# ZhengyiLuo/PULSE

Hardware: AMD Instinct MI355X
Metric: env-steps/sec through PPO update (higher is better)
Workload: dtype f32; 1 GPU; cfg2: 4096 SMPL-humanoid envs/GPU x horizon 32, imitation obs/reward/reset + PPO (actor+critic MLP [1024, 512], minibatch 16384 x 6 mini-epochs); num_envs_per_gpu=4096, horizon=32, global_batch=131072, parallelism=dp1, reference_motion=HBM-resident motion library (1024 clips), queried every step

## Files before the change

pulse_amd/csrc/build.py:

```python
import argparse
import os
import subprocess
from concurrent.futures import ThreadPoolExecutor

HERE = os.path.dirname(os.path.abspath(__file__))
ROOT = os.path.dirname(os.path.dirname(HERE))
INCLUDE = os.path.join(ROOT, "include")
LIB = os.path.join(HERE, "libpulse_hip.so")
ARCH = "gfx950"

NO_CONTRACT = ["-ffp-contract=off"]
NO_PACKED_F32 = ["-fno-slp-vectorize", "-fno-vectorize"]
LLVM_BIN = "/opt/rocm/lib/llvm/bin"
SOURCES = [
    ("capi.cpp", []),
    ("rot_ops.hip", NO_CONTRACT),
    ("env_step.hip", NO_CONTRACT),
    ("amp_obs.hip", NO_CONTRACT),
    ("task_step.hip", NO_CONTRACT),
    ("traj_step.hip", NO_CONTRACT),
    ("motion_state.hip", NO_CONTRACT),
    ("motion_build.hip", NO_CONTRACT),
    ("eval_metrics.hip", NO_CONTRACT),
    ("rollout_ops.hip", NO_CONTRACT),
    ("gae.hip", NO_CONTRACT),
    ("gemm_f32.hip", ["-mllvm", "-amdgpu-mfma-vgpr-form"]),
    ("gemm_x3.hip", ["-mllvm", "-amdgpu-mfma-vgpr-form"]),
    ("gemm_api.hip", ["-mllvm", "-amdgpu-mfma-vgpr-form"]),
    ("gemm_x3p.hip", ["-mllvm", "-amdgpu-mfma-vgpr-form"]),
    ("gemm_b16.hip", ["-mllvm", "-amdgpu-mfma-vgpr-form"]),
    ("gemm_x3p_api.hip", ["-mllvm", "-amdgpu-mfma-vgpr-form"]),
    ("gemm_x3w.hip", ["-mllvm", "-pragma-unroll-threshold=4000000", "-Wno-unused-const-variable"]),
    ("gemm_x3s.hip", ["-mllvm", "-amdgpu-mfma-vgpr-form"]),
    ("learner_ops.hip", NO_CONTRACT),
    ("b16_ops.hip", NO_CONTRACT),
    ("vae_head.hip", NO_CONTRACT),
    ("mcp.hip", NO_CONTRACT),
]


def hipcc():
    for cand in (os.environ.get("HIPCC"), "/opt/rocm/bin/hipcc", "hipcc"):
        if cand and (os.path.isabs(cand) and os.path.exists(cand) or not os.path.isabs(cand)):
            return cand
    raise RuntimeError("hipcc not found")


HOST_ONLY_OBJECTS = ("capi.o",)


def llvm_bin():
    cc = hipcc()
    cands = []
    if os.path.isabs(cc):
        cands.append(os.path.join(os.path.dirname(os.path.dirname(os.path.realpath(cc))), "lib", "llvm", "bin"))
    cands.append(LLVM_BIN)
    for c in cands:
        if os.path.exists(os.path.join(c, "llvm-objdump")):
            return c
    raise RuntimeError("llvm-objdump / llvm-objcopy / clang-offload-bundler not found next to hipcc: the device-ISA audit cannot run")


def packed_f32_instructions(obj, host_only=False):
    import re
    import tempfile
    with tempfile.TemporaryDirectory() as tmp:
        fat, co = os.path.join(tmp, "fat"), os.path.join(tmp, "co")
        llvm = llvm_bin()
        r = subprocess.run([f"{llvm}/llvm-objcopy", "--dump-section", f".hip_fatbin={fat}", obj], capture_output=True, text=True)
        if r.returncode != 0 or not os.path.exists(fat) or os.path.getsize(fat) == 0:
            if host_only:
                return []
            raise RuntimeError(f"{obj}: no .hip_fatbin section could be extracted ({r.stderr.strip() or 'empty section'}); cannot audit its device ISA")
        subprocess.run([f"{llvm}/clang-offload-bundler", "--unbundle", "--type=o", f"--targets=hipv4-amdgcn-amd-amdhsa--{ARCH}",
                        f"--input={fat}", f"--output={co}"], check=True, capture_output=True)
        if not os.path.exists(co) or os.path.getsize(co) == 0:
            raise RuntimeError(f"{obj}: the offload bundle holds no {ARCH} code object; cannot audit its device ISA")
        dis = subprocess.run([f"{llvm}/llvm-objdump", "-d", co], check=True, capture_output=True, text=True).stdout
    return re.findall(r"\bv_pk_(?:mul|add|fma)_f32\b[^\n]*", dis)


def _newer(a, b):
    return (not os.path.exists(b)) or os.path.getmtime(a) > os.path.getmtime(b)


def build(force=False, verbose=False):
    cc = hipcc()
    headers = [os.path.join(HERE, f) for f in os.listdir(HERE) if f.endswith(".h")]
    headers.append(os.path.join(INCLUDE, "pulse_hip.h"))
    headers.append(os.path.abspath(__file__))
    common = ["-x", "hip", f"--offload-arch={ARCH}", "-O3", "-std=c++17", "-fPIC", "-Wall",
              "-Wno-unused-function", f"-I{INCLUDE}", f"-I{HERE}"] + NO_PACKED_F32
    jobs = []
    objs = []
    for src, extra in SOURCES:
        s = os.path.join(HERE, src)
        if not os.path.exists(s):
            continue
        o = os.path.join(HERE, os.path.splitext(src)[0] + ".o")
        objs.append(o)
        if force or _newer(s, o) or any(_newer(h, o) for h in headers):
            jobs.append((src, [cc] + common + extra + ["-c", s, "-o", o]))

    def run(job):
        name, cmd = job
        if verbose:
            print(" ".join(cmd), flush=True)
        r = subprocess.run(cmd, stdout=subprocess.PIPE, stderr=subprocess.STDOUT, text=True)
        return name, r.returncode, r.stdout

    with ThreadPoolExecutor(max_workers=max(1, min(len(jobs), os.cpu_count() or 1))) as ex:
        for name, rc, out in ex.map(run, jobs):
            if out.strip() and (verbose or rc != 0):
                print(f"--- {name} ---\n{out}", flush=True)
            if rc != 0:
                raise RuntimeError(f"hipcc failed on {name}")
    for o in objs:
        bad = packed_f32_instructions(o, host_only=os.path.basename(o) in HOST_ONLY_OBJECTS)
        if bad:
            raise RuntimeError(f"{os.path.basename(o)}: {len(bad)} packed-fp32 VALU instructions in the device code (e.g. {bad[0].strip()}); "
                               "they are unsafe beside MFMA waves on gfx950 (see the note at the top of build.py)")
    if jobs or force or not os.path.exists(LIB) or any(_newer(o, LIB) for o in objs):
        cmd = [cc, "-shared", "-fPIC", f"--offload-arch={ARCH}", "-o", LIB] + objs
        if verbose:
            print(" ".join(cmd), flush=True)
        r = subprocess.run(cmd, stdout=subprocess.PIPE, stderr=subprocess.STDOUT, text=True)
        if r.returncode != 0:
            print(r.stdout)
            raise RuntimeError("link failed")
    return LIB


if __name__ == "__main__":
    ap = argparse.ArgumentParser()
    ap.add_argument("--force", action="store_true")
    ap.add_argument("--verbose", action="store_true")
    a = ap.parse_args()
    print(build(a.force, a.verbose))
```

pulse_amd/csrc/gemm_api.hip:

```cpp
#include <cstdlib>
#include "common.h"
#include "gemm_shared.h"

namespace pulse {

__global__ void __launch_bounds__(256) reduce_slabs_kernel(const float* __restrict__ slabs, int nslab, long long slab_stride,
                                                          long long count, float* __restrict__ out, float scale) {
    for (long long i = ((long long)blockIdx.x * blockDim.x + threadIdx.x) * 4; i < count; i += (long long)gridDim.x * blockDim.x * 4) {
        if (i + 3 < count) {
            float4 s = *reinterpret_cast<const float4*>(slabs + i);
            float4 s1 = make_float4(0.f, 0.f, 0.f, 0.f), s2 = s1, s3 = s1;
            int k = 1;
            for (; k + 15 < nslab; k += 16) {
                float4 v[16];
#pragma unroll
                for (int u = 0; u < 16; ++u) v[u] = *reinterpret_cast<const float4*>(slabs + (k + u) * slab_stride + i);
#pragma unroll
                for (int u = 0; u < 16; u += 4) {
                    s.x += v[u].x; s.y += v[u].y; s.z += v[u].z; s.w += v[u].w;
                    s1.x += v[u + 1].x; s1.y += v[u + 1].y; s1.z += v[u + 1].z; s1.w += v[u + 1].w;
                    s2.x += v[u + 2].x; s2.y += v[u + 2].y; s2.z += v[u + 2].z; s2.w += v[u + 2].w;
                    s3.x += v[u + 3].x; s3.y += v[u + 3].y; s3.z += v[u + 3].z; s3.w += v[u + 3].w;
                }
            }
            for (; k + 3 < nslab; k += 4) {
                const float4 v0 = *reinterpret_cast<const float4*>(slabs + k * slab_stride + i);
                const float4 v1 = *reinterpret_cast<const float4*>(slabs + (k + 1) * slab_stride + i);
                const float4 v2 = *reinterpret_cast<const float4*>(slabs + (k + 2) * slab_stride + i);
                const float4 v3 = *reinterpret_cast<const float4*>(slabs + (k + 3) * slab_stride + i);
                s.x += v0.x; s.y += v0.y; s.z += v0.z; s.w += v0.w;
                s1.x += v1.x; s1.y += v1.y; s1.z += v1.z; s1.w += v1.w;
                s2.x += v2.x; s2.y += v2.y; s2.z += v2.z; s2.w += v2.w;
                s3.x += v3.x; s3.y += v3.y; s3.z += v3.z; s3.w += v3.w;
            }
            const int rem = nslab - k;
            if (rem == 3) {
                const float4 t0 = *reinterpret_cast<const float4*>(slabs + k * slab_stride + i);
                const float4 t1 = *reinterpret_cast<const float4*>(slabs + (k + 1) * slab_stride + i);
                const float4 t2 = *reinterpret_cast<const float4*>(slabs + (k + 2) * slab_stride + i);
                s.x += t0.x; s.y += t0.y; s.z += t0.z; s.w += t0.w;
                s.x += t1.x; s.y += t1.y; s.z += t1.z; s.w += t1.w;
                s.x += t2.x; s.y += t2.y; s.z += t2.z; s.w += t2.w;
            } else if (rem == 2) {
                const float4 t0 = *reinterpret_cast<const float4*>(slabs + k * slab_stride + i);
                const float4 t1 = *reinterpret_cast<const float4*>(slabs + (k + 1) * slab_stride + i);
                s.x += t0.x; s.y += t0.y; s.z += t0.z; s.w += t0.w;
                s.x += t1.x; s.y += t1.y; s.z += t1.z; s.w += t1.w;
            } else if (rem == 1) {
                const float4 t0 = *reinterpret_cast<const float4*>(slabs + k * slab_stride + i);
                s.x += t0.x; s.y += t0.y; s.z += t0.z; s.w += t0.w;
            }
            s.x = (s.x + s1.x) + (s2.x + s3.x); s.y = (s.y + s1.y) + (s2.y + s3.y); s.z = (s.z + s1.z) + (s2.z + s3.z); s.w = (s.w + s1.w) + (s2.w + s3.w);
            s.x *= scale; s.y *= scale; s.z *= scale; s.w *= scale;
            *reinterpret_cast<float4*>(out + i) = s;
        } else {
            for (long long e = i; e < count; ++e) {
                float s = slabs[e];
                for (int k = 1; k < nslab; ++k) s += slabs[k * slab_stride + e];
                out[e] = s * scale;
            }
        }
    }
}

__global__ void __launch_bounds__(256) colsum_partial_kernel(const float* __restrict__ X, int M, int N, int ld, int rows_per_chunk,
                                                            float* __restrict__ partial, long long ldp) {
    __shared__ float4 red[4][64];
    const int cg = threadIdx.x & 63, rl = threadIdx.x >> 6;
    const int c = blockIdx.x * 256 + cg * 4;
    const int r0 = blockIdx.y * rows_per_chunk;
    const int r1 = min(M, r0 + rows_per_chunk);
    float4 s0 = make_float4(0.f, 0.f, 0.f, 0.f), s1 = s0, s2 = s0, s3 = s0;
    if (c < N) {
        const float* p = X + c;
        int r = r0 + rl;
        for (; r + 12 < r1; r += 16) {
            const float4 a = *reinterpret_cast<const float4*>(p + (long long)r * ld);
            const float4 b = *reinterpret_cast<const float4*>(p + (long long)(r + 4) * ld);
            const float4 cc = *reinterpret_cast<const float4*>(p + (long long)(r + 8) * ld);
            const float4 d = *reinterpret_cast<const float4*>(p + (long long)(r + 12) * ld);
            s0.x += a.x; s0.y += a.y; s0.z += a.z; s0.w += a.w;
            s1.x += b.x; s1.y += b.y; s1.z += b.z; s1.w += b.w;
            s2.x += cc.x; s2.y += cc.y; s2.z += cc.z; s2.w += cc.w;
            s3.x += d.x; s3.y += d.y; s3.z += d.z; s3.w += d.w;
        }
        for (; r < r1; r += 4) {
            const float4 a = *reinterpret_cast<const float4*>(p + (long long)r * ld);
            s0.x += a.x; s0.y += a.y; s0.z += a.z; s0.w += a.w;
        }
    }
    s0.x += s1.x + s2.x + s3.x; s0.y += s1.y + s2.y + s3.y; s0.z += s1.z + s2.z + s3.z; s0.w += s1.w + s2.w + s3.w;
    red[rl][cg] = s0;
    __syncthreads();
    if (rl == 0 && c < N) {
        const float4 a = red[0][cg], b = red[1][cg], cc = red[2][cg], d = red[3][cg];
        float* o = partial + (long long)blockIdx.y * ldp + c;
        o[0] = a.x + b.x + cc.x + d.x;
        if (c + 1 < N) o[1] = a.y + b.y + cc.y + d.y;
        if (c + 2 < N) o[2] = a.z + b.z + cc.z + d.z;
        if (c + 3 < N) o[3] = a.w + b.w + cc.w + d.w;
    }
}

}

using namespace pulse;

namespace {
thread_local long long* g_dbg = nullptr;
thread_local int g_last_tile = 0;
thread_local int g_opt[16] = {0, 0, 0, 0, 0, 0, 0, 0, 0, 0, 0, 0, 0, 0, 0, 0};
}

namespace pulse { int gemm_option(int key) { return key >= 0 && key < 16 ? g_opt[key] : 0; } long long* gemm_debug_buffer() { return g_dbg; } }

namespace {
constexpr int WIDE_TILE = 256;
bool skinny_env_off() { static const bool off = [] { const char* e = getenv("PULSE_X3_SKINNY"); return e && e[0] == '0'; }(); return off; }
bool g_skinny_unavailable = false;
bool g_wide_unavailable = false;
int x3_mode() {
    static const int env = [] { const char* e = getenv("PULSE_X3_WIDE"); return e ? atoi(e) : -1; }();
    int mode = g_opt[4];
    if (mode == 0 && env >= 0) mode = env == 0 ? 1 : env == 1 ? 0 : env;
    return g_wide_unavailable ? 1 : mode;
}
bool x3_wide_tile(const GemmArgs& g, int lda, int ldb, bool akc, bool bkc) {
    const int mode = x3_mode();
    if (mode == 1 || g.M <= 128 || g.N <= 128) return false;
    if ((long long)lda * (akc ? 257 : g.kchunk + 1) >= (1LL << 28) || (long long)ldb * (bkc ? 257 : g.kchunk + 1) >= (1LL << 28) ||
        (long long)g.ldc * 257 >= (1LL << 28) || (long long)g.ldaux * 257 >= (1LL << 28))
        return false;
    if (mode == 2) return true;
    const long long z = (long long)g.batch * g.splitk;
    const long long nt = (long long)((g.M + 127) / 128) * ((g.N + 127) / 128) * z;
    const long long wt = (long long)((g.M + 255) / 256) * ((g.N + 255) / 256) * z;
    const long long rem = nt % 512;
    const double cost_narrow = 2.0 * (double)(nt / 512) + (rem == 0 ? 0.0 : rem <= 256 ? 1.5 : 2.0);
    const double kk = (double)g.kchunk < (double)g.K ? (double)g.kchunk : (double)g.K;
    const double fw = g.epi == 2 ? 45.0 : (g.epi == 0 && g.act >= 2) ? 30.0 : 8.0;
    const double wide_round = 2.0 * (0.1526 * kk + fw) / (0.0924 * kk + 5.0);
    const double cost_wide = wide_round * (double)((wt + 255) / 256);
    return cost_wide < cost_narrow;
}
}

extern "C" {

int pulse_sizeof_gemm_desc(void) { return (int)sizeof(pulse_gemm_desc); }

int pulse_gemm_set_debug_buffer(long long* device_buffer) { g_dbg = device_buffer; return PULSE_OK; }

int pulse_gemm_last_tile(void) { return g_last_tile; }
int pulse_gemm_x3_mode(void) { return x3_mode(); }

int pulse_gemm_set_option(int key, int value) {
    PULSE_REQUIRE(key >= 0 && key < 16, "pulse_gemm_set_option: bad key");
    g_opt[key] = value;
    return PULSE_OK;
}

int pulse_gemm_f32(const pulse_gemm_desc* d, pulse_stream_t s) {
    PULSE_REQUIRE(d != nullptr, "pulse_gemm_f32: null descriptor");
    PULSE_REQUIRE(d->M >= 0 && d->N >= 0 && d->K >= 0, "pulse_gemm_f32: negative size");
    if (d->M == 0 || d->N == 0 || d->batch == 0) return PULSE_OK;
    PULSE_REQUIRE(d->A && d->B && d->C, "pulse_gemm_f32: null operand");
    PULSE_REQUIRE(d->batch >= 1 && d->split_k >= 1, "pulse_gemm_f32: batch / split_k must be >= 1");
    PULSE_REQUIRE((d->lda % 4) == 0 && (d->ldb % 4) == 0, "pulse_gemm_f32: lda / ldb must be multiples of 4 floats");
    PULSE_REQUIRE((reinterpret_cast<uintptr_t>(d->A) & 15) == 0 && (reinterpret_cast<uintptr_t>(d->B) & 15) == 0,
                  "pulse_gemm_f32: A / B must be 16-byte aligned");
    PULSE_REQUIRE((d->stride_a % 4) == 0 && (d->stride_b % 4) == 0, "pulse_gemm_f32: batch strides must be multiples of 4 floats");
    const bool akc = d->a_layout == PULSE_GEMM_RED_CONTIG, bkc = d->b_layout == PULSE_GEMM_RED_CONTIG;
    PULSE_REQUIRE(!(!akc && bkc), "pulse_gemm_f32: layout combination (A out-contiguous, B reduction-contiguous) unsupported");
    const int k4 = (d->K + 3) & ~3;
    PULSE_REQUIRE(akc ? d->lda >= k4 : d->lda >= ((d->M + 3) & ~3), "pulse_gemm_f32: lda too small");
    PULSE_REQUIRE(bkc ? d->ldb >= k4 : d->ldb >= ((d->N + 3) & ~3), "pulse_gemm_f32: ldb too small");
    PULSE_REQUIRE(d->ldc >= d->N, "pulse_gemm_f32: ldc too small");
    PULSE_REQUIRE(d->epilogue >= 0 && d->epilogue <= 3 && d->activation >= 0 && d->activation <= 3, "pulse_gemm_f32: bad epilogue / activation");
    PULSE_REQUIRE(d->activation != PULSE_ACT_SILU_D || (d->C2 != nullptr && d->ldc2 >= d->N), "pulse_gemm_f32: ACT_SILU_D stores the derivative in C2");
    PULSE_REQUIRE(d->epilogue == 0 || d->activation == 0, "pulse_gemm_f32: a gradient epilogue takes no activation");
    PULSE_REQUIRE(d->epilogue == 0 || d->aux != nullptr || (d->epilogue == PULSE_EPI_RELU_GRAD && d->relu_mask != nullptr),
                  "pulse_gemm_f32: gradient epilogue needs aux (or, for relu-grad, relu_mask)");
    const bool mask_on = d->relu_mask != nullptr && ((d->epilogue == PULSE_EPI_RELU_GRAD && d->aux == nullptr) ||
                                                     (d->epilogue == PULSE_EPI_BIAS_ACT && d->activation == PULSE_ACT_RELU));
    PULSE_REQUIRE(!mask_on || (d->ld_mask >= (d->N + 3) / 4 && d->split_k == 1), "pulse_gemm_f32: relu_mask needs ld_mask >= roundup4(N) / 4 and no split-K");
    PULSE_REQUIRE(d->rowsum == nullptr || (!akc && !bkc), "pulse_gemm_f32: rowsum needs the (OUT, OUT) layouts (dW pass)");
    PULSE_REQUIRE(d->split_k == 1 || (d->epilogue == 0 && d->activation == 0 && d->bias == nullptr),
                  "pulse_gemm_f32: split-K slabs carry no epilogue");

    GemmArgs g;
    g.A = d->A; g.B = d->B; g.C = d->C; g.C2 = d->C2; g.bias = d->bias; g.aux = d->aux;
    g.M = d->M; g.N = d->N; g.K = d->K;
    g.lda = d->lda; g.ldb = d->ldb; g.ldc = d->ldc; g.ldc2 = d->ldc2; g.ldaux = d->ldaux;
    g.sA = d->stride_a; g.sB = d->stride_b; g.sC = d->stride_c; g.sC2 = d->stride_c2; g.sBias = d->stride_bias; g.sAux = d->stride_aux;
    g.batch = d->batch; g.splitk = d->split_k;
    const int bk = d->compute_type == PULSE_GEMM_COMPUTE_BF16 ? BK16 : d->compute_type == PULSE_GEMM_COMPUTE_F32X3 ? XK : BK;
    int kchunk = (d->K + d->split_k - 1) / d->split_k;
    kchunk = ((kchunk + bk - 1) / bk) * bk;
    g.kchunk = kchunk > 0 ? kchunk : bk;
    g.sSplit = d->split_stride;
    g.act = d->activation; g.epi = d->epilogue;
    g.rowsum = d->rowsum; g.sRowsum = d->stride_rowsum;
    g.mask = mask_on ? d->relu_mask : nullptr; g.ldmask = d->ld_mask; g.sMask = d->stride_mask;
    g.tiles_m = (d->M + BM - 1) / BM; g.tiles_n = (d->N + BN - 1) / BN;
    const bool half_tile = d->compute_type == PULSE_GEMM_COMPUTE_F32X3 && d->M >= 256 && g.tiles_n == 1 &&
                           (long long)g.tiles_m * d->batch * d->split_k < 384 && g_opt[2] == 0;
    if (half_tile) g.tiles_m = (d->M + 63) / 64;
    g.dbg = g_dbg;
    PULSE_REQUIRE(d->compute_type == PULSE_GEMM_COMPUTE_F32 || d->compute_type == PULSE_GEMM_COMPUTE_BF16 ||
                  d->compute_type == PULSE_GEMM_COMPUTE_F32X3, "pulse_gemm_f32: bad compute_type");
    const bool bf = d->compute_type == PULSE_GEMM_COMPUTE_BF16, x3 = d->compute_type == PULSE_GEMM_COMPUTE_F32X3;
    g.round_bf16 = bf && d->round_output_bf16 ? 1 : 0;
    PULSE_REQUIRE((long long)d->lda * (akc ? 129 : g.kchunk + 1) < (1LL << 28) && (long long)d->ldb * (bkc ? 129 : g.kchunk + 1) < (1LL << 28) &&
                  (long long)d->ldc * 129 < (1LL << 28) && (long long)d->ldaux * 129 < (1LL << 28),
                  "pulse_gemm_f32: pitch too large for 32-bit tile-relative offsets");
    auto al16 = [](const void* p, long long ld, long long st) { return (reinterpret_cast<uintptr_t>(p) & 15) == 0 && (ld % 4) == 0 && (st % 4) == 0; };
    g.vec_epi = al16(d->C, d->ldc, d->stride_c) && (d->split_stride % 4) == 0 && (!d->aux || al16(d->aux, d->ldaux, d->stride_aux)) &&
                (!d->C2 || al16(d->C2, d->ldc2, d->stride_c2)) && (!d->bias || al16(d->bias, 4, d->stride_bias));
    PULSE_REQUIRE(!mask_on || g.vec_epi, "pulse_gemm_f32: relu_mask needs 16-byte aligned C / pitches (a lane owns four columns of a mask word)");
    g_last_tile = half_tile ? 64 : 128;
    if (x3 && akc && d->N <= 96 && d->epilogue == PULSE_EPI_BIAS_ACT && d->activation <= PULSE_ACT_RELU && d->C2 == nullptr && d->split_k == 1 &&
        d->rowsum == nullptr && !mask_on && g_dbg == nullptr && g_opt[6] == 0 && !g_skinny_unavailable && !skinny_env_off() &&
        (long long)((d->M + 127) / 128) * d->batch >= 192 && (long long)((d->M + 127) / 128) * d->batch <= 256 && (long long)d->lda * 129 < (1LL << 28) &&
        (bkc ? (long long)d->ldb * 97 : (long long)d->ldb * (d->K + 1)) < (1LL << 28)) {
        const int rc = launch_gemm_x3s(g, bkc, as_stream(s));
        if (rc != kWideTileUnavailable) { g_last_tile = 96; return rc; }
        g_skinny_unavailable = true;
    }
    if (x3 && !half_tile && x3_wide_tile(g, d->lda, d->ldb, akc, bkc)) {
        const int ntail = d->N % WIDE_TILE;
        if (ntail > 0 && ntail <= 64 && d->N > WIDE_TILE && d->split_k == 1 && d->rowsum == nullptr && g_opt[5] == 0) {
            const long long tm = (d->M + WIDE_TILE - 1) / WIDE_TILE, z = d->batch;
            const long long r_all = (tm * ((d->N + WIDE_TILE - 1) / WIDE_TILE) * z + 255) / 256, r_main = (tm * (d->N / WIDE_TILE) * z + 255) / 256;
            if (r_main < r_all) {
                const int n0 = d->N - ntail;
                pulse_gemm_desc m = *d, t = *d;
                m.N = n0;
                t.N = ntail;
                t.B = bkc ? d->B + (long long)n0 * d->ldb : d->B + n0;
                t.C = d->C + n0;
                if (d->C2) t.C2 = d->C2 + n0;
                if (d->bias) t.bias = d->bias + n0;
                if (d->aux) t.aux = d->aux + n0;
                if (d->relu_mask) t.relu_mask = d->relu_mask + n0 / 4;
                const int rc_main = pulse_gemm_f32(&m, s);
                if (rc_main != PULSE_OK) return rc_main;
                const int rc_tail = pulse_gemm_f32(&t, s);
                g_last_tile = 256;
                return rc_tail;
            }
        }
        const int rc = launch_gemm_x3w(g, akc, bkc, as_stream(s));
        if (rc != kWideTileUnavailable) { g_last_tile = 256; return rc; }
        g_wide_unavailable = true;
    }
    const size_t extra_lds = (size_t)g_opt[1];
    if (x3) return launch_gemm_x3(g, akc, bkc, half_tile, extra_lds, as_stream(s));
    if (bf) return launch_gemm_bf16c(g, akc, bkc, extra_lds, as_stream(s));
    return launch_gemm_mfma32(g, akc, bkc, extra_lds, as_stream(s));
}

int pulse_reduce_slabs(const float* slabs, int32_t num_slabs, int64_t slab_stride, int64_t count, float* out, float scale,
                       pulse_stream_t s) {
    PULSE_REQUIRE(num_slabs >= 1 && count >= 0, "pulse_reduce_slabs: bad sizes");
    if (count == 0) return PULSE_OK;
    PULSE_REQUIRE(slabs && out, "pulse_reduce_slabs: null pointer");
    PULSE_REQUIRE((slab_stride % 4) == 0 && (reinterpret_cast<uintptr_t>(slabs) & 15) == 0 && (reinterpret_cast<uintptr_t>(out) & 15) == 0,
                  "pulse_reduce_slabs: 16-byte alignment required");
    long long blocks = (count / 4 + 255) / 256;
    if (blocks > 2048) blocks = 2048;
    if (blocks < 1) blocks = 1;
    hipLaunchKernelGGL(reduce_slabs_kernel, dim3((unsigned)blocks), dim3(256), 0, as_stream(s), slabs, num_slabs, slab_stride, count, out, scale);
    return check_launch("pulse_reduce_slabs");
}

int pulse_colsum_partial(const float* x, int32_t m, int32_t n, int32_t ld, int32_t num_chunks, float* partial, int64_t ld_partial,
                         pulse_stream_t s) {
    PULSE_REQUIRE(m >= 0 && n >= 0 && num_chunks >= 1, "pulse_colsum_partial: bad sizes");
    if (n == 0) return PULSE_OK;
    PULSE_REQUIRE(x && partial && ld >= ((n + 3) & ~3) && ld_partial >= n, "pulse_colsum_partial: bad pointers / pitches (ld must cover roundup4(n))");
    PULSE_REQUIRE((ld % 4) == 0 && (reinterpret_cast<uintptr_t>(x) & 15) == 0, "pulse_colsum_partial: x rows must be 16-byte aligned");
    const int rows = (m + num_chunks - 1) / num_chunks;
    hipLaunchKernelGGL(colsum_partial_kernel, dim3((unsigned)((n + 255) / 256), (unsigned)num_chunks), dim3(256), 0, as_stream(s), x, m, n, ld,
                       rows > 0 ? rows : 1, partial, (long long)ld_partial);
    return check_launch("pulse_colsum_partial");
}
}
```

pulse_amd/csrc/gemm_shared.h:

```cpp
#pragma once
#include "common.h"

namespace pulse {

typedef float f32x16 __attribute__((ext_vector_type(16)));
typedef float f32x4 __attribute__((ext_vector_type(4)));
typedef unsigned int u32x4 __attribute__((ext_vector_type(4)));

constexpr unsigned RSRC_FLAGS = 0x00020000u;

struct GemmArgs {
    const float* A; const float* B; float* C; float* C2; const float* bias; const float* aux;
    int M, N, K;
    int lda, ldb, ldc, ldc2, ldaux;
    long long sA, sB, sC, sC2, sBias, sAux;
    int batch, splitk, kchunk;
    long long sSplit;
    int act;
    int epi;
    int tiles_m, tiles_n;
    int vec_epi;
    float* rowsum; long long sRowsum;
    long long* dbg;
    int round_bf16;
    unsigned* mask; int ldmask; long long sMask;
};

__device__ __forceinline__ long long mask_word(int r, int cg, int ldmask) { return (long long)((r >> 6) * 8 + (r & 7)) * ldmask + cg; }

constexpr int BM = 128, BN = 128;
constexpr int BK = 32, BK16 = 64, XK = 16;
constexpr int CP = BN;

constexpr int kWideTileUnavailable = -1000;

__device__ __forceinline__ int slot_of(int out) { return out ^ ((out >> 3) & 7); }

__device__ __forceinline__ f32x4 buf_load(__amdgpu_buffer_rsrc_t r, int voff, int soff) {
    return __builtin_bit_cast(f32x4, __builtin_amdgcn_raw_buffer_load_b128(r, voff, soff, 0));
}
__device__ __forceinline__ void buf_store(f32x4 v, __amdgpu_buffer_rsrc_t r, int voff, int soff) {
    __builtin_amdgcn_raw_buffer_store_b128(__builtin_bit_cast(u32x4, v), r, voff, soff, 0);
}
__device__ __forceinline__ f32x4 lds_read(int byte_addr) {
    extern __shared__ __attribute__((aligned(16))) char smem_c[];
    return *reinterpret_cast<const f32x4*>(smem_c + byte_addr);
}
__device__ __forceinline__ void lds_write(int byte_addr, f32x4 v) {
    extern __shared__ __attribute__((aligned(16))) char smem_c[];
    *reinterpret_cast<f32x4*>(smem_c + byte_addr) = v;
}

typedef __bf16 bf16x2 __attribute__((ext_vector_type(2)));
typedef __bf16 bf16x8 __attribute__((ext_vector_type(8)));
typedef float f32x2 __attribute__((ext_vector_type(2)));

__device__ __forceinline__ unsigned fbits(float v) { return __builtin_bit_cast(unsigned, v); }
__device__ __forceinline__ float bitsf(unsigned v) { return __builtin_bit_cast(float, v); }
__device__ __forceinline__ unsigned pack_rn(float lo_elem, float hi_elem) {
    return __builtin_bit_cast(unsigned, __builtin_convertvector((f32x2){lo_elem, hi_elem}, bf16x2));
}

__device__ __forceinline__ float silu(float z) { return z / (1.f + __expf(-z)); }
__device__ __forceinline__ float silu_deriv(float z) {
    const float sg = 1.f / (1.f + __expf(-z));
    return sg * (1.f + z * (1.f - sg));
}
__device__ __forceinline__ float rbf(float v) { return (float)(__bf16)v; }

inline int lds_launch_status(hipError_t e, const char* what) {
    if (e != hipSuccess) return fail(PULSE_ERR_LAUNCH, "%s: LDS attribute: %s", what, hipGetErrorString(e));
    return check_launch(what);
}

int launch_gemm_mfma32(const GemmArgs& g, bool akc, bool bkc, size_t extra_lds, hipStream_t stream);
int launch_gemm_bf16c(const GemmArgs& g, bool akc, bool bkc, size_t extra_lds, hipStream_t stream);
int launch_gemm_x3(const GemmArgs& g, bool akc, bool bkc, bool half_tile, size_t extra_lds, hipStream_t stream);
int launch_gemm_x3w(const GemmArgs& g, bool akc, bool bkc, hipStream_t stream);
int launch_gemm_x3s(const GemmArgs& g, bool bkc, hipStream_t stream);

}
```

Baseline: 1.931 million env-steps/s.

## Add skinny-M split-bf16x3 MFMA kernel for small-M head weight gradients

Adds a dedicated GEMM kernel for products with M<=96 and N a multiple of 32. It targets the backward weight gradients of the small output heads. Three waves split A into three bf16 parts and stage them in double-buffered LDS, while all waves stream B through registers and issue 32x32x16 bf16 MFMAs for a six-term split product that keeps fp32-like accuracy. The dispatcher routes qualifying launches with 192-256 workgroups to this kernel and falls back if the launch fails. This replaces a generic tiled kernel that wastes most of a 128-row tile on small M, at the cost of extra code paths and a fragile dispatch condition.

```diff
diff --git a/pulse_amd/csrc/build.py b/pulse_amd/csrc/build.py
--- a/pulse_amd/csrc/build.py
+++ b/pulse_amd/csrc/build.py
@@ -32,6 +32,7 @@
     ("gemm_x3p_api.hip", ["-mllvm", "-amdgpu-mfma-vgpr-form"]),
     ("gemm_x3w.hip", ["-mllvm", "-pragma-unroll-threshold=4000000", "-Wno-unused-const-variable"]),
     ("gemm_x3s.hip", ["-mllvm", "-amdgpu-mfma-vgpr-form"]),
+    ("gemm_x3sm.hip", []),
     ("learner_ops.hip", NO_CONTRACT),
     ("b16_ops.hip", NO_CONTRACT),
     ("vae_head.hip", NO_CONTRACT),
diff --git a/pulse_amd/csrc/gemm_api.hip b/pulse_amd/csrc/gemm_api.hip
--- a/pulse_amd/csrc/gemm_api.hip
+++ b/pulse_amd/csrc/gemm_api.hip
@@ -118,6 +118,8 @@
 constexpr int WIDE_TILE = 256;
 bool skinny_env_off() { static const bool off = [] { const char* e = getenv("PULSE_X3_SKINNY"); return e && e[0] == '0'; }(); return off; }
 bool g_skinny_unavailable = false;
+bool heads_bwd_env_off() { static const bool off = [] { const char* e = getenv("PULSE_X3_HEADS_BWD"); return e && e[0] == '0'; }(); return off; }
+bool g_skinny_m_unavailable = false;
 bool g_wide_unavailable = false;
 int x3_mode() {
     static const int env = [] { const char* e = getenv("PULSE_X3_WIDE"); return e ? atoi(e) : -1; }();
@@ -227,6 +229,15 @@
         if (rc != kWideTileUnavailable) { g_last_tile = 96; return rc; }
         g_skinny_unavailable = true;
     }
+    if (x3 && !akc && !bkc && d->M <= 96 && (d->N % 32) == 0 && d->epilogue == PULSE_EPI_BIAS_ACT && d->activation == PULSE_ACT_NONE &&
+        d->bias == nullptr && d->C2 == nullptr && !mask_on && g_dbg == nullptr && g_opt[10] != 1 && !heads_bwd_env_off() && !g_skinny_m_unavailable) {
+        const long long nwg = (long long)((d->N + 127) / 128) * d->batch * d->split_k;
+        if (g_opt[10] == 2 ? nwg < (1LL << 31) : (nwg >= 192 && nwg <= 256)) {
+            const int rc = launch_gemm_x3sm(g, as_stream(s));
+            if (rc != kWideTileUnavailable) { g_last_tile = 97; return rc; }
+            g_skinny_m_unavailable = true;
+        }
+    }
     if (x3 && !half_tile && x3_wide_tile(g, d->lda, d->ldb, akc, bkc)) {
         const int ntail = d->N % WIDE_TILE;
         if (ntail > 0 && ntail <= 64 && d->N > WIDE_TILE && d->split_k == 1 && d->rowsum == nullptr && g_opt[5] == 0) {
diff --git a/pulse_amd/csrc/gemm_shared.h b/pulse_amd/csrc/gemm_shared.h
--- a/pulse_amd/csrc/gemm_shared.h
+++ b/pulse_amd/csrc/gemm_shared.h
@@ -78,5 +78,6 @@
 int launch_gemm_x3(const GemmArgs& g, bool akc, bool bkc, bool half_tile, size_t extra_lds, hipStream_t stream);
 int launch_gemm_x3w(const GemmArgs& g, bool akc, bool bkc, hipStream_t stream);
 int launch_gemm_x3s(const GemmArgs& g, bool bkc, hipStream_t stream);
+int launch_gemm_x3sm(const GemmArgs& g, hipStream_t stream);
 
 }
diff --git a/pulse_amd/csrc/gemm_x3sm.hip b/pulse_amd/csrc/gemm_x3sm.hip
--- /dev/null
+++ b/pulse_amd/csrc/gemm_x3sm.hip
@@ -0,0 +1,257 @@
+#include <type_traits>
+#include "gemm_shared.h"
+
+namespace pulse {
+
+constexpr int W_MT = 3;
+constexpr int W_COLS = 128;
+constexpr int W_FRAG = 64 * 16;
+constexpr int W_STAGERS = 2 * 32 * W_MT;
+
+struct SplitW {
+    u32x4 p0, p1, p2;
+    __device__ __forceinline__ void pair(const float (&v)[8], int k) {
+        const float a = v[2 * k], b = v[2 * k + 1];
+        const unsigned q0 = pack_rn(a, b);
+        p0[k] = q0;
+        const float ra = a - bitsf(q0 << 16), rb = b - bitsf(q0 & 0xffff0000u);
+        const unsigned q1 = pack_rn(ra, rb);
+        p1[k] = q1;
+        const float sa = ra - bitsf(q1 << 16), sb = rb - bitsf(q1 & 0xffff0000u);
+        p2[k] = pack_rn(sa, sb);
+    }
+    __device__ __forceinline__ void run(const float (&v)[8]) {
+#pragma unroll
+        for (int k = 0; k < 4; ++k) pair(v, k);
+    }
+};
+
+template <int STEPS>
+__global__ void __launch_bounds__(256) __attribute__((amdgpu_waves_per_eu(1, 1))) gemm_x3sm_kernel(const GemmArgs g) {
+    constexpr int KP = 16 * STEPS;
+    constexpr int STAGE = STEPS * W_MT * 3 * W_FRAG;
+    extern __shared__ __attribute__((aligned(16))) char smem_c[];
+    const int tid = threadIdx.x;
+    const int lane = tid & 63;
+    const int wave = __builtin_amdgcn_readfirstlane(tid >> 6);
+    const int half = lane >> 5, l31 = lane & 31;
+    const int ncb = (g.N + W_COLS - 1) / W_COLS;
+    const int nslab = g.batch * g.splitk;
+    int cb, slab;
+    if ((nslab & 7) == 0) {
+        const int q = blockIdx.x >> 3;
+        cb = q % ncb;
+        slab = (q / ncb) * 8 + (blockIdx.x & 7);
+    } else {
+        cb = blockIdx.x % ncb;
+        slab = blockIdx.x / ncb;
+    }
+    const int sp = slab % g.splitk, bz = slab / g.splitk;
+    const int n0 = cb * W_COLS;
+    const int kbeg = sp * g.kchunk;
+    const int klen = min(g.K, kbeg + g.kchunk) - kbeg;
+    if (klen <= 0) {
+        float* C0 = g.C + bz * g.sC + sp * g.sSplit;
+        const int c0 = n0 + (tid & 127);
+        if (c0 < g.N)
+            for (int r = tid >> 7; r < g.M; r += 2) C0[(long long)r * g.ldc + c0] = 0.f;
+        if (g.rowsum != nullptr && cb == 0 && tid < g.M) g.rowsum[bz * g.sRowsum + sp * g.sSplit + tid] = 0.f;
+        return;
+    }
+    const int nph = (klen + KP - 1) / KP;
+    const int klast = klen - 1;
+
+    const float* Ab = g.A + bz * g.sA + (long long)kbeg * g.lda;
+    const float* Bb = g.B + bz * g.sB + (long long)kbeg * g.ldb;
+    const unsigned recA = (unsigned)((klen - 1) * g.lda + g.M) * 4u;
+    const unsigned recB = (unsigned)((klen - 1) * g.ldb + g.N) * 4u;
+    const __amdgpu_buffer_rsrc_t rsA = __builtin_amdgcn_make_buffer_rsrc(const_cast<float*>(Ab), 0, recA, RSRC_FLAGS);
+    const __amdgpu_buffer_rsrc_t rsB = __builtin_amdgcn_make_buffer_rsrc(const_cast<float*>(Bb), 0, recB, RSRC_FLAGS);
+    const int ld4A = g.lda * 4, ld4B = g.ldb * 4;
+
+    const int voB = (8 * half * g.ldb + n0 + 32 * wave + l31) * 4;
+    float hw[STEPS][8];
+    auto load_h = [&](auto clamp_tag, int s, int kbase) {
+        int so = (kbase + 16 * s) * ld4B;
+#pragma unroll
+        for (int e = 0; e < 8; ++e) {
+            if constexpr (decltype(clamp_tag)::value) so = min(kbase + 16 * s + e, klast) * ld4B;
+            hw[s][e] = bitsf(__builtin_amdgcn_raw_buffer_load_b32(rsB, voB, so, 0));
+            so += ld4B;
+            asm volatile("" : "+s"(so));
+        }
+    };
+
+    const bool stager = wave < W_MT;
+    const int zh = tid >= 32 * W_MT ? 1 : 0, zm = tid - 32 * W_MT * zh;
+    const int voA = stager ? (8 * zh * g.lda + zm) * 4 : 0x40000000;
+    const int ldsA = stager ? ((zm >> 5) * 3) * W_FRAG + (zh * 32 + (zm & 31)) * 16 : 2 * STAGE + lane * 16;
+    const int zmul = stager ? 1 : 0;
+    float zraw[STEPS][8];
+    auto load_z = [&](auto clamp_tag, int s, int kbase) {
+        int so = (kbase + 16 * s) * ld4A;
+#pragma unroll
+        for (int e = 0; e < 8; ++e) {
+            if constexpr (decltype(clamp_tag)::value) so = min(kbase + 16 * s + e, klast) * ld4A;
+            zraw[s][e] = bitsf(__builtin_amdgcn_raw_buffer_load_b32(rsA, voA, so, 0));
+            so += ld4A;
+            asm volatile("" : "+s"(so));
+        }
+    };
+    auto mask_z = [&](int s, int kbase) {
+#pragma unroll
+        for (int e = 0; e < 8; ++e)
+            if (kbase + 16 * s + 8 * zh + e >= klen) zraw[s][e] = 0.f;
+    };
+    float rs_acc = 0.f;
+    const bool do_rs = g.rowsum != nullptr && cb == 0;
+    auto sum_z = [&](int s, bool tile_exists) {
+        const float t = ((zraw[s][0] + zraw[s][1]) + (zraw[s][2] + zraw[s][3])) + ((zraw[s][4] + zraw[s][5]) + (zraw[s][6] + zraw[s][7]));
+        rs_acc = tile_exists ? rs_acc + t : rs_acc;
+    };
+
+    f32x16 acc[W_MT];
+#pragma unroll
+    for (int i = 0; i < W_MT; ++i)
+#pragma unroll
+        for (int r = 0; r < 16; ++r) acc[i][r] = 0.f;
+
+    using T = std::true_type; using F = std::false_type;
+#pragma unroll
+    for (int s = 0; s < STEPS; ++s) load_h(T{}, s, 0);
+#pragma unroll
+    for (int s = 0; s < STEPS; ++s) load_z(T{}, s, 0);
+#pragma unroll
+    for (int s = 0; s < STEPS; ++s) {
+        mask_z(s, 0);
+        sum_z(s, 16 * s < klen);
+        SplitW sp3;
+        sp3.run(zraw[s]);
+        char* dst = smem_c + zmul * s * (W_MT * 3 * W_FRAG) + ldsA;
+        *reinterpret_cast<u32x4*>(dst) = sp3.p0;
+        *reinterpret_cast<u32x4*>(dst + W_FRAG) = sp3.p1;
+        *reinterpret_cast<u32x4*>(dst + 2 * W_FRAG) = sp3.p2;
+    }
+#pragma unroll
+    for (int s = 0; s < STEPS; ++s) load_z(T{}, s, KP);
+    __syncthreads();
+
+    auto phase = [&](auto more_tag, auto tail_tag, auto next_tail_tag, auto load2_tag, int p) {
+        constexpr bool MORE = decltype(more_tag)::value, TAIL = decltype(tail_tag)::value, NEXT_TAIL = decltype(next_tail_tag)::value;
+        constexpr int LOAD2 = decltype(load2_tag)::value;
+        const int kbase = p * KP;
+        const int cur = (p & 1) * STAGE;
+        SplitW fh;
+        if constexpr (TAIL) {
+#pragma unroll
+            for (int e = 0; e < 8; ++e)
+                if (kbase + 8 * half + e >= klen) hw[0][e] = 0.f;
+        }
+        fh.run(hw[0]);
+        bf16x8 fz[2][W_MT][3];
+        SplitW fn, sz;
+        auto frag = [&](auto set_tag, int s, int u) {
+            constexpr int SET = decltype(set_tag)::value;
+            const int i = u / 3, pl = u % 3;
+            fz[SET][i][pl] = *reinterpret_cast<const bf16x8*>(smem_c + cur + ((s * W_MT + i) * 3 + pl) * W_FRAG + lane * 16);
+        };
+        using S0 = std::integral_constant<int, 0>; using S1 = std::integral_constant<int, 1>;
+#pragma unroll
+        for (int u = 0; u < 9; ++u) frag(S0{}, 0, u);
+#pragma unroll
+        for (int s = 0; s < STEPS; ++s) {
+            const int k0 = kbase + 16 * s;
+            const bool live = !TAIL || k0 < klen;
+            const bf16x8 h0 = __builtin_bit_cast(bf16x8, fh.p0), h1 = __builtin_bit_cast(bf16x8, fh.p1), h2 = __builtin_bit_cast(bf16x8, fh.p2);
+            const bool nxt = s + 1 < STEPS;
+            if (nxt) {
+                if constexpr (TAIL) {
+#pragma unroll
+                    for (int e = 0; e < 8; ++e)
+                        if (k0 + 16 + 8 * half + e >= klen) hw[s + 1][e] = 0.f;
+                }
+            }
+#pragma unroll
+            for (int q = 0; q < 6 * W_MT; ++q) {
+                if (live) {
+                    const int term = q / W_MT, i = q % W_MT, sq = s & 1;
+                    const bf16x8 av = term == 0 ? fz[sq][i][2] : (term == 2 || term == 3) ? fz[sq][i][1] : fz[sq][i][0];
+                    const bf16x8 bv = term == 1 ? h2 : (term == 2 || term == 4) ? h1 : h0;
+                    acc[i] = __builtin_amdgcn_mfma_f32_32x32x16_bf16(av, bv, acc[i], 0, 0, 0);
+                }
+                if (nxt && q < 8 && (q & 1) == 0) fn.pair(hw[s + 1], q >> 1);
+                if (q == 0) {
+                    if constexpr (MORE) load_h(std::integral_constant<bool, NEXT_TAIL>{}, s, kbase + KP);
+                }
+                if (nxt && (q & 1) == 1 && q < 10) {
+                    const int u0 = q - 1;
+                    if (s & 1) { frag(S0{}, s + 1, u0); if (u0 + 1 < 9) frag(S0{}, s + 1, u0 + 1); }
+                    else { frag(S1{}, s + 1, u0); if (u0 + 1 < 9) frag(S1{}, s + 1, u0 + 1); }
+                }
+                if constexpr (MORE) {
+                    if (q == 8) {
+                        if constexpr (NEXT_TAIL) mask_z(s, kbase + KP);
+                        sum_z(s, !NEXT_TAIL || k0 + KP < klen);
+                    }
+                    if (q >= 8 && q < 16 && (q & 1) == 0) sz.pair(zraw[s], (q - 8) >> 1);
+                    char* dst = smem_c + zmul * (((p + 1) & 1) * STAGE + s * (W_MT * 3 * W_FRAG)) + ldsA;
+                    if (q == 15) *reinterpret_cast<u32x4*>(dst) = sz.p0;
+                    if (q == 16) *reinterpret_cast<u32x4*>(dst + W_FRAG) = sz.p1;
+                    if (q == 17) {
+                        *reinterpret_cast<u32x4*>(dst + 2 * W_FRAG) = sz.p2;
+                        if constexpr (LOAD2 == 1) load_z(std::false_type{}, s, kbase + 2 * KP);
+                        if constexpr (LOAD2 == 2) load_z(std::true_type{}, s, kbase + 2 * KP);
+                    }
+                }
+                __builtin_amdgcn_sched_barrier(0);
+            }
+            if (nxt) fh = fn;
+        }
+        __syncthreads();
+    };
+    const bool ktail = (klen % KP) != 0;
+    using L0 = std::integral_constant<int, 0>; using L1 = std::integral_constant<int, 1>; using L2 = std::integral_constant<int, 2>;
+    for (int p = 0; p + 3 < nph; ++p) phase(T{}, F{}, F{}, L1{}, p);
+    if (nph > 2) {
+        if (ktail) phase(T{}, F{}, F{}, L2{}, nph - 3);
+        else phase(T{}, F{}, F{}, L1{}, nph - 3);
+    }
+    if (nph > 1) {
+        if (ktail) phase(T{}, F{}, T{}, L0{}, nph - 2);
+        else phase(T{}, F{}, F{}, L0{}, nph - 2);
+    }
+    if (ktail) phase(F{}, T{}, F{}, L0{}, nph - 1);
+    else phase(F{}, F{}, F{}, L0{}, nph - 1);
+
+    if (do_rs) {
+        float* sm = reinterpret_cast<float*>(smem_c);
+        if (tid < W_STAGERS) sm[tid] = rs_acc;
+        __syncthreads();
+        if (tid < 32 * W_MT && tid < g.M) g.rowsum[bz * g.sRowsum + sp * g.sSplit + tid] = sm[tid] + sm[tid + 32 * W_MT];
+    }
+
+    float* C = g.C + bz * g.sC + sp * g.sSplit;
+    const int col = n0 + 32 * wave + l31;
+    if (col < g.N) {
+#pragma unroll
+        for (int i = 0; i < W_MT; ++i) {
+#pragma unroll
+            for (int r = 0; r < 16; ++r) {
+                const int row = 32 * i + (r & 3) + 8 * (r >> 2) + 4 * half;
+                if (row < g.M) C[(long long)row * g.ldc + col] = acc[i][r];
+            }
+        }
+    }
+}
+
+constexpr int W_STEPS = 4;
+constexpr int W_LDS = 2 * W_STEPS * W_MT * 3 * W_FRAG + 3 * W_FRAG;
+
+int launch_gemm_x3sm(const GemmArgs& g, hipStream_t stream) {
+    const dim3 grid((unsigned)(((g.N + W_COLS - 1) / W_COLS) * g.batch * g.splitk)), block(256);
+    const hipError_t e = launch_dyn_lds<gemm_x3sm_kernel<W_STEPS>>(grid, block, W_LDS, stream, g);
+    if (e != hipSuccess) { (void)hipGetLastError(); return kWideTileUnavailable; }
+    return check_launch("pulse_gemm_f32 (skinny-M weight gradient)");
+}
+
+}
```

Measured after the change: 1.925 million env-steps/s, median of 2. No clear change (-0.3%).

## Add short-M weight-gradient GEMM kernel for small output heads

Applied to the files above, without the earlier changes.

Adds a dedicated bf16x3-split MFMA kernel for weight-gradient GEMMs whose M is at most 96 (such as the small policy and value heads). Each workgroup holds the whole short M extent and 128 columns, double-buffers K in LDS and prefetches the next phase into registers. It can also accumulate the bias rowsum in the same pass. The kernel is dispatched when the workgroup count and K chunk fit a heuristic window, and the build step now checks that it uses no scratch or VGPR spills. The aim is to stop padding these skinny GEMMs to 128-row tiles; the cost is more code and a forced one-wave-per-EU occupancy.

```diff
diff --git a/pulse_amd/csrc/build.py b/pulse_amd/csrc/build.py
--- a/pulse_amd/csrc/build.py
+++ b/pulse_amd/csrc/build.py
@@ -32,6 +32,7 @@
     ("gemm_x3p_api.hip", ["-mllvm", "-amdgpu-mfma-vgpr-form"]),
     ("gemm_x3w.hip", ["-mllvm", "-pragma-unroll-threshold=4000000", "-Wno-unused-const-variable"]),
     ("gemm_x3s.hip", ["-mllvm", "-amdgpu-mfma-vgpr-form"]),
+    ("gemm_x3m.hip", []),
     ("learner_ops.hip", NO_CONTRACT),
     ("b16_ops.hip", NO_CONTRACT),
     ("vae_head.hip", NO_CONTRACT),
@@ -45,6 +46,8 @@
             return cand
     raise RuntimeError("hipcc not found")
 
+
+NO_SPILL_KERNELS = {"gemm_x3m.o": ("gemm_x3m_kernel",)}
 
 HOST_ONLY_OBJECTS = ("capi.o",)
 
@@ -78,6 +81,36 @@
             raise RuntimeError(f"{obj}: the offload bundle holds no {ARCH} code object; cannot audit its device ISA")
         dis = subprocess.run([f"{llvm}/llvm-objdump", "-d", co], check=True, capture_output=True, text=True).stdout
     return re.findall(r"\bv_pk_(?:mul|add|fma)_f32\b[^\n]*", dis)
+
+
+def kernel_resources(obj):
+    import re
+    import tempfile
+    with tempfile.TemporaryDirectory() as tmp:
+        fat, co = os.path.join(tmp, "fat"), os.path.join(tmp, "co")
+        llvm = llvm_bin()
+        subprocess.run([f"{llvm}/llvm-objcopy", "--dump-section", f".hip_fatbin={fat}", obj], check=True, capture_output=True)
+        subprocess.run([f"{llvm}/clang-offload-bundler", "--unbundle", "--type=o", f"--targets=hipv4-amdgcn-amd-amdhsa--{ARCH}",
+                        f"--input={fat}", f"--output={co}"], check=True, capture_output=True)
+        notes = subprocess.run([f"{llvm}/llvm-readelf", "--notes", co], check=True, capture_output=True, text=True).stdout
+    out = {}
+    for block in re.split(r"\n\s*- (?=\.)", notes):
+        name = re.search(r"\.name:\s*(\S+)", block)
+        if name and ".private_segment_fixed_size" in block:
+            out[name.group(1)] = {k: int(v) for k, v in re.findall(r"\.(\w+):\s*(\d+)\s*$", block, flags=re.M)}
+    return out
+
+
+def check_no_spill(obj, kernels):
+    res = kernel_resources(obj)
+    for want in kernels:
+        hits = {n: r for n, r in res.items() if want in n}
+        if not hits:
+            raise RuntimeError(f"{os.path.basename(obj)}: no kernel named *{want}* in the code object's metadata")
+        for n, r in hits.items():
+            if r.get("private_segment_fixed_size", -1) != 0 or r.get("vgpr_spill_count", -1) != 0:
+                raise RuntimeError(f"{os.path.basename(obj)}: {n} uses {r.get('private_segment_fixed_size')} B of scratch and spills "
+                                   f"{r.get('vgpr_spill_count')} VGPRs; it must use none")
 
 
 def _newer(a, b):
@@ -120,6 +153,9 @@
         if bad:
             raise RuntimeError(f"{os.path.basename(o)}: {len(bad)} packed-fp32 VALU instructions in the device code (e.g. {bad[0].strip()}); "
                                "they are unsafe beside MFMA waves on gfx950 (see the note at the top of build.py)")
+    for o in objs:
+        if os.path.basename(o) in NO_SPILL_KERNELS:
+            check_no_spill(o, NO_SPILL_KERNELS[os.path.basename(o)])
     if jobs or force or not os.path.exists(LIB) or any(_newer(o, LIB) for o in objs):
         cmd = [cc, "-shared", "-fPIC", f"--offload-arch={ARCH}", "-o", LIB] + objs
         if verbose:
diff --git a/pulse_amd/csrc/gemm_api.hip b/pulse_amd/csrc/gemm_api.hip
--- a/pulse_amd/csrc/gemm_api.hip
+++ b/pulse_amd/csrc/gemm_api.hip
@@ -117,6 +117,9 @@
 namespace {
 constexpr int WIDE_TILE = 256;
 bool skinny_env_off() { static const bool off = [] { const char* e = getenv("PULSE_X3_SKINNY"); return e && e[0] == '0'; }(); return off; }
+bool heads_grad_env_off() { static const bool off = [] { const char* e = getenv("PULSE_X3_HEADS_GRAD"); return e && e[0] == '0'; }(); return off; }
+bool g_short_m_unavailable = false;
+int heads_grad_mode() { const int o = g_opt[10]; return o == 0 && heads_grad_env_off() ? 1 : o; }
 bool g_skinny_unavailable = false;
 bool g_wide_unavailable = false;
 int x3_mode() {
@@ -227,6 +230,15 @@
         if (rc != kWideTileUnavailable) { g_last_tile = 96; return rc; }
         g_skinny_unavailable = true;
     }
+    if (x3 && !akc && !bkc && d->M <= 96 && d->epilogue == PULSE_EPI_BIAS_ACT && d->activation == PULSE_ACT_NONE && d->bias == nullptr &&
+        d->C2 == nullptr && !mask_on && g_dbg == nullptr && heads_grad_mode() != 1 && !g_short_m_unavailable) {
+        const long long nwg = (long long)g.tiles_n * d->batch * d->split_k;
+        if (heads_grad_mode() == 2 || (nwg >= 128 && nwg <= 256 && g.kchunk >= 128 && d->M > 32)) {
+            const int rc = launch_gemm_x3m(g, as_stream(s));
+            if (rc != kWideTileUnavailable) { g_last_tile = 97; return rc; }
+            g_short_m_unavailable = true;
+        }
+    }
     if (x3 && !half_tile && x3_wide_tile(g, d->lda, d->ldb, akc, bkc)) {
         const int ntail = d->N % WIDE_TILE;
         if (ntail > 0 && ntail <= 64 && d->N > WIDE_TILE && d->split_k == 1 && d->rowsum == nullptr && g_opt[5] == 0) {
diff --git a/pulse_amd/csrc/gemm_shared.h b/pulse_amd/csrc/gemm_shared.h
--- a/pulse_amd/csrc/gemm_shared.h
+++ b/pulse_amd/csrc/gemm_shared.h
@@ -78,5 +78,6 @@
 int launch_gemm_x3(const GemmArgs& g, bool akc, bool bkc, bool half_tile, size_t extra_lds, hipStream_t stream);
 int launch_gemm_x3w(const GemmArgs& g, bool akc, bool bkc, hipStream_t stream);
 int launch_gemm_x3s(const GemmArgs& g, bool bkc, hipStream_t stream);
+int launch_gemm_x3m(const GemmArgs& g, hipStream_t stream);
 
 }
diff --git a/pulse_amd/csrc/gemm_x3m.hip b/pulse_amd/csrc/gemm_x3m.hip
--- /dev/null
+++ b/pulse_amd/csrc/gemm_x3m.hip
@@ -0,0 +1,258 @@
+#include <type_traits>
+#include "gemm_shared.h"
+
+namespace pulse {
+
+constexpr int M_NT = 3;
+constexpr int M_COLS = 128;
+constexpr int M_KP = 128;
+constexpr int M_STEPS = M_KP / 16;
+constexpr int M_FRAG = 64 * 16;
+constexpr int M_FRAGS = M_STEPS * M_NT * 3 * M_FRAG;
+constexpr int M_RS = (M_KP / 8) * 96 * 4;
+constexpr int M_STAGE = M_FRAGS + M_RS;
+constexpr int M_LDS = 2 * M_STAGE;
+constexpr int M_UNITS = M_NT * 32 * (M_KP / 8) / 256;
+constexpr int M_LEAD = 3;
+constexpr int M_OOR = 0x40000000;
+
+struct SplitM8 {
+    u32x4 p0, p1, p2;
+    __device__ __forceinline__ void pair(const float (&v)[8], int k) {
+        const float a = v[2 * k], b = v[2 * k + 1];
+        const unsigned q0 = pack_rn(a, b);
+        p0[k] = q0;
+        const float ra = a - bitsf(q0 << 16), rb = b - bitsf(q0 & 0xffff0000u);
+        const unsigned q1 = pack_rn(ra, rb);
+        p1[k] = q1;
+        const float sa = ra - bitsf(q1 << 16), sb = rb - bitsf(q1 & 0xffff0000u);
+        p2[k] = pack_rn(sa, sb);
+    }
+    __device__ __forceinline__ void run(const float (&v)[8]) {
+#pragma unroll
+        for (int k = 0; k < 4; ++k) pair(v, k);
+    }
+};
+
+__global__ void __launch_bounds__(256) __attribute__((amdgpu_waves_per_eu(1, 1))) gemm_x3m_kernel(const GemmArgs g) {
+    extern __shared__ __attribute__((aligned(16))) char smem_c[];
+    const int tid = threadIdx.x;
+    const int lane = tid & 63;
+    const int wave = __builtin_amdgcn_readfirstlane(tid >> 6);
+    const int half = lane >> 5, l31 = lane & 31;
+    const WgMap wg = map_workgroup(g.tiles_n, g.batch, g.splitk);
+    const int n0 = wg.id * M_COLS;
+    const int bz = wg.bz, sp = wg.sp;
+    const int kbeg = sp * g.kchunk;
+    const int klen = min(g.K, kbeg + g.kchunk) - kbeg;
+    const int nph = klen > 0 ? (klen + M_KP - 1) / M_KP : 0;
+
+    const int extA = g.M, extB = min(M_COLS, g.N - n0);
+    const float* Ab = g.A + bz * g.sA + (long long)kbeg * g.lda;
+    const float* Bb = g.B + bz * g.sB + (long long)kbeg * g.ldb + n0;
+    const unsigned recA = klen > 0 ? (unsigned)((klen - 1) * g.lda + extA) * 4u : 0u;
+    const unsigned recB = klen > 0 ? (unsigned)((klen - 1) * g.ldb + extB) * 4u : 0u;
+    const __amdgpu_buffer_rsrc_t rsA = __builtin_amdgcn_make_buffer_rsrc(const_cast<float*>(Ab), 0, recA, RSRC_FLAGS);
+    const __amdgpu_buffer_rsrc_t rsB = __builtin_amdgcn_make_buffer_rsrc(const_cast<float*>(Bb), 0, recB, RSRC_FLAGS);
+    const int ldb4 = g.ldb * 4, lda4 = g.lda * 4;
+
+    const int voB = wave * 32 + l31 < extB ? (8 * half * g.ldb + wave * 32 + l31) * 4 : M_OOR;
+    float b[M_STEPS][8];
+    auto load_b = [&](auto guard_tag, int s, int kbase) {
+        const int left = klen - (kbase + 16 * s + 8 * half);
+        int so = (kbase + 16 * s) * ldb4;
+        asm volatile("" : "+s"(so));
+#pragma unroll
+        for (int e = 0; e < 8; ++e) {
+            int vo = voB;
+            if constexpr (decltype(guard_tag)::value) vo = e < left ? voB : M_OOR;
+            b[s][e] = bitsf(__builtin_amdgcn_raw_buffer_load_b32(rsB, vo, so, 0));
+            so += ldb4;
+        }
+    };
+
+    float araw[M_UNITS][8];
+    const int kgl = tid >> 5, ml = tid & 31;
+    const int a_vo = (8 * kgl * g.lda + ml) * 4;
+    const int a_lds = ((kgl >> 1) * M_NT * 3) * M_FRAG + ((kgl & 1) * 32 + ml) * 16;
+    const int a_rs = M_FRAGS + (kgl * 96 + ml) * 4;
+    auto lds_of = [&](int u) { return a_lds + ((4 * (u & 1) * M_NT + (u >> 1)) * 3) * M_FRAG; };
+    auto rs_of = [&](int u) { return a_rs + (8 * (u & 1) * 96 + 32 * (u >> 1)) * 4; };
+    auto left_of = [&](int u, int kbase) {
+        return 32 * (u >> 1) + ml < extA ? klen - (kbase + 8 * kgl + 64 * (u & 1)) : 0;
+    };
+    auto load_a = [&](int u, int kbase) {
+        const int left = left_of(u, kbase);
+        int so = (kbase + 64 * (u & 1)) * lda4 + 32 * (u >> 1) * 4;
+        asm volatile("" : "+s"(so));
+#pragma unroll
+        for (int e = 0; e < 8; ++e) {
+            araw[u][e] = bitsf(__builtin_amdgcn_raw_buffer_load_b32(rsA, e < left ? a_vo : M_OOR, so, 0));
+            so += lda4;
+        }
+    };
+    auto sum8 = [&](int u) { return ((araw[u][0] + araw[u][1]) + (araw[u][2] + araw[u][3])) + ((araw[u][4] + araw[u][5]) + (araw[u][6] + araw[u][7])); };
+    auto mask_a = [&](int u, int kbase) {
+        const int left = left_of(u, kbase);
+#pragma unroll
+        for (int e = 0; e < 8; ++e)
+            if (e >= left) araw[u][e] = 0.f;
+    };
+
+    f32x16 acc[M_NT];
+#pragma unroll
+    for (int j = 0; j < M_NT; ++j)
+#pragma unroll
+        for (int r = 0; r < 16; ++r) acc[j][r] = 0.f;
+    float rs_acc = 0.f;
+    const bool do_rs = g.rowsum != nullptr && wg.id == 0;
+    const int rs_rd = M_FRAGS + tid * 4;
+
+    if (nph > 0) {
+#pragma unroll
+        for (int s = 0; s < M_STEPS; ++s) load_b(std::true_type{}, s, 0);
+#pragma unroll
+        for (int u = 0; u < M_UNITS; ++u) load_a(u, 0);
+#pragma unroll
+        for (int u = 0; u < M_UNITS; ++u) {
+            mask_a(u, 0);
+            SplitM8 sx;
+            sx.run(araw[u]);
+            char* dst = smem_c + lds_of(u);
+            *reinterpret_cast<u32x4*>(dst) = sx.p0;
+            *reinterpret_cast<u32x4*>(dst + M_FRAG) = sx.p1;
+            *reinterpret_cast<u32x4*>(dst + 2 * M_FRAG) = sx.p2;
+            *reinterpret_cast<float*>(smem_c + rs_of(u)) = sum8(u);
+        }
+        if (nph > 1) {
+#pragma unroll
+            for (int u = 0; u < M_UNITS - M_LEAD; ++u) load_a(u, M_KP);
+        }
+    }
+    __syncthreads();
+
+    auto phase = [&](auto more_tag, auto tail_tag, auto next_tail_tag, int p) {
+        constexpr bool MORE = decltype(more_tag)::value, TAIL = decltype(tail_tag)::value, NEXT_TAIL = decltype(next_tail_tag)::value;
+        const int kbase = p * M_KP;
+        const int cur = (p & 1) * M_STAGE;
+        if (do_rs && tid < 192) {
+#pragma unroll
+            for (int t = 0; t < M_STEPS; ++t) rs_acc += *reinterpret_cast<const float*>(smem_c + cur + rs_rd + t * 2 * 96 * 4);
+        }
+        SplitM8 fa;
+        if constexpr (TAIL) {
+#pragma unroll
+            for (int e = 0; e < 8; ++e)
+                if (kbase + 8 * half + e >= klen) b[0][e] = 0.f;
+        }
+        fa.run(b[0]);
+        bf16x8 fr0[2][M_NT], fr1[M_NT], fr2[M_NT];
+        SplitM8 fn, sx;
+        auto rd = [&](int s, int j, int pl) {
+            return *reinterpret_cast<const bf16x8*>(smem_c + cur + ((s * M_NT + j) * 3 + pl) * M_FRAG + lane * 16);
+        };
+#pragma unroll
+        for (int j = 0; j < M_NT; ++j) { fr2[j] = rd(0, j, 2); fr0[0][j] = rd(0, j, 0); fr1[j] = rd(0, j, 1); }
+#pragma unroll
+        for (int s = 0; s < M_STEPS; ++s) {
+            const int k0 = kbase + 16 * s;
+            const bool live = !TAIL || k0 < klen;
+            const bf16x8 b0 = __builtin_bit_cast(bf16x8, fa.p0), b1 = __builtin_bit_cast(bf16x8, fa.p1), b2 = __builtin_bit_cast(bf16x8, fa.p2);
+            const bool nxt = s + 1 < M_STEPS;
+            const bool stg = MORE && s < M_UNITS;
+            const int sq = s & 1;
+            if (nxt) {
+                if constexpr (TAIL) {
+#pragma unroll
+                    for (int e = 0; e < 8; ++e)
+                        if (k0 + 16 + 8 * half + e >= klen) b[s + 1][e] = 0.f;
+                }
+            }
+            float rs8 = 0.f;
+            if constexpr (MORE) {
+                if (stg) {
+                    if constexpr (NEXT_TAIL) mask_a(s, kbase + M_KP);
+                    rs8 = sum8(s);
+                }
+            }
+#pragma unroll
+            for (int q = 0; q < 6 * M_NT; ++q) {
+                if (live) {
+                    const int term = q / M_NT, j = q % M_NT;
+                    const bf16x8 av = term == 0 ? fr2[j] : (term == 2 || term == 3) ? fr1[j] : fr0[sq][j];
+                    const bf16x8 bv = term == 1 ? b2 : (term == 2 || term == 4) ? b1 : b0;
+                    acc[j] = __builtin_amdgcn_mfma_f32_32x32x16_bf16(av, bv, acc[j], 0, 0, 0);
+                }
+                if (nxt && q < 8 && (q & 1) == 0) fn.pair(b[s + 1], q >> 1);
+                if (q == 0) { if constexpr (MORE) load_b(next_tail_tag, s, kbase + M_KP); }
+                if (nxt) {
+                    if (q == 3) { fr2[0] = rd(s + 1, 0, 2); fr2[1] = rd(s + 1, 1, 2); }
+                    if (q == 5) { fr2[2] = rd(s + 1, 2, 2); fr0[sq ^ 1][0] = rd(s + 1, 0, 0); }
+                    if (q == 7) { fr0[sq ^ 1][1] = rd(s + 1, 1, 0); fr0[sq ^ 1][2] = rd(s + 1, 2, 0); }
+                    if (q == 11) { fr1[0] = rd(s + 1, 0, 1); fr1[1] = rd(s + 1, 1, 1); }
+                    if (q == 13) fr1[2] = rd(s + 1, 2, 1);
+                }
+                if constexpr (MORE) {
+                    if (stg) {
+                        if (q >= 8 && q < 16 && (q & 1) == 0) sx.pair(araw[s], (q - 8) >> 1);
+                        char* nst = smem_c + ((p + 1) & 1) * M_STAGE;
+                        char* dst = nst + lds_of(s);
+                        if (q == 15) *reinterpret_cast<u32x4*>(dst) = sx.p0;
+                        if (q == 16) *reinterpret_cast<u32x4*>(dst + M_FRAG) = sx.p1;
+                        if (q == 17) {
+                            *reinterpret_cast<u32x4*>(dst + 2 * M_FRAG) = sx.p2;
+                            *reinterpret_cast<float*>(nst + rs_of(s)) = rs8;
+                        }
+                    }
+                    if (q == 17) {
+                        if (s + M_LEAD < M_UNITS) load_a(s + M_LEAD, kbase + M_KP);
+                        else if (s >= M_STEPS - M_LEAD) load_a(s - (M_STEPS - M_LEAD), kbase + 2 * M_KP);
+                    }
+                }
+                __builtin_amdgcn_sched_barrier(0);
+            }
+            if (nxt) fa = fn;
+        }
+        __syncthreads();
+    };
+    using T = std::true_type; using F = std::false_type;
+    const bool ktail = (klen % M_KP) != 0;
+    for (int p = 0; p + 2 < nph; ++p) phase(T{}, F{}, F{}, p);
+    if (nph > 1) {
+        if (ktail) phase(T{}, F{}, T{}, nph - 2);
+        else phase(T{}, F{}, F{}, nph - 2);
+    }
+    if (nph > 0) {
+        if (ktail) phase(F{}, T{}, F{}, nph - 1);
+        else phase(F{}, F{}, F{}, nph - 1);
+    }
+
+    if (do_rs) {
+        float* ex = reinterpret_cast<float*>(smem_c);
+        if (tid < 192) ex[tid] = rs_acc;
+        __syncthreads();
+        if (tid < 96 && tid < g.M) g.rowsum[bz * g.sRowsum + sp * g.sSplit + tid] = ex[tid] + ex[tid + 96];
+    }
+
+    float* C = g.C + bz * g.sC + sp * g.sSplit;
+    const int col = n0 + wave * 32 + l31;
+    if (col < g.N) {
+#pragma unroll
+        for (int j = 0; j < M_NT; ++j) {
+#pragma unroll
+            for (int r = 0; r < 16; ++r) {
+                const int row = 32 * j + (r & 3) + 8 * (r >> 2) + 4 * half;
+                if (row < g.M) C[(long long)row * g.ldc + col] = acc[j][r];
+            }
+        }
+    }
+}
+
+int launch_gemm_x3m(const GemmArgs& g, hipStream_t stream) {
+    const dim3 grid((unsigned)g.tiles_n, (unsigned)(g.batch * g.splitk)), block(256);
+    const hipError_t e = launch_dyn_lds<gemm_x3m_kernel>(grid, block, M_LDS, stream, g);
+    if (e != hipSuccess) { (void)hipGetLastError(); return kWideTileUnavailable; }
+    return check_launch("pulse_gemm_f32 (short-M weight-gradient tile)");
+}
+
+}
```

Measured after the change: 1.934 million env-steps/s before, 1.955 million env-steps/s after (median of 4 runs). 1.01x the previous value.
